# khanhptnk/psketch

Measured on AMD Instinct MI355X. Metric: env-steps/sec (whole node), 12x12 craft_medium, batch=65536, higher is better.
Workload: dtype fp32; 1 GPU; craft_medium_12x12_w3_B65536_random_rollout_full_features_K32; world=craft_medium_12x12, envs_per_gpu=65536, global_batch=65536, window=3, n_features=404, obs_dtype=fp32, state_dtype=u8 (exact small integers; the reference's float64 arrays hold the same values), obs_ring=16, pool=1024, parallelism=env-shard x1, ticks_per_launch=32, launches=81, teach_table=auto, obs_store=sc1, tile=32, rollout_threads=512

## Files before the change

psketch_amd/csrc/craft_episode.h:

```cpp
#pragma once
#include "craft_device.h"

namespace craft {


__device__ __forceinline__ int hashed_action(const SimView& v, uint64_t seed, int64_t slot, int64_t tick) {
  const uint64_t gid = (uint64_t)(v.env_base + slot);
  return (int)((uint32_t)(splitmix64(seed ^ (gid << 20) ^ (uint64_t)tick) >> 32) % 6u);
}

__device__ __forceinline__ bool state_in_range(const SimView& v, const Agent& s) {
  return !(s.x < 1 || s.x > v.W - 2 || s.y < 1 || s.y > v.H - 2 || s.scen >= v.pool_count);
}

__device__ __forceinline__ void protocol_step(Agent& s, const int& act, const uint32_t& flags, int& d, int& counted, bool& restart) {
  if (s.frozen) {
    d = 1;
  } else {
    counted = 1;
    s.timer -= 1;
    d = (act == CRAFT_STOP) || s.timer <= 0;
    restart = d && (flags & CRAFT_STEP_AUTORESET);
  }
}

__device__ __forceinline__ void language_step_begin(const Agent& s, const int& act, int& d, int& counted, bool& bad) {
  if (s.frozen) {
    d = 1;
  } else {
    bad = act < 0 || act >= CRAFT_N_ACTIONS;
    counted = !bad;
  }
}
__device__ __forceinline__ void language_step_end(Agent& s, const int& act, int& d) {
  s.timer -= 1;
  d = (act == CRAFT_STOP) || s.timer <= 0;
  if (d) {
    s.frozen = 1;
    s.timer = max(s.timer, 0);
  }
}

__device__ __forceinline__ void restart_agent(Agent& s, uint32_t init_word, int maxT) {
  s.x = init_word & 0xff; s.y = (init_word >> 8) & 0xff; s.dir = (init_word >> 16) & 3;
  s.timer = maxT;
}

__device__ __forceinline__ int32_t queue_next(int32_t cur, const uint32_t& count, const uint32_t& step, const uint32_t& wrap) {
  if (cur < 0) return -1;
  uint32_t nx = (uint32_t)cur + step;
  if (nx >= count) {
    if (!wrap) return -1;
    nx -= count;
  }
  return (int32_t)nx;
}

__device__ __forceinline__ bool episode_ends(const Agent& s, int act) {
  return !s.frozen && (act == CRAFT_STOP || s.timer <= 1);
}

__device__ __forceinline__ bool language_episode_ends(const Agent& s, int act) {
  return !s.frozen && act >= 0 && act < CRAFT_N_ACTIONS && (act == CRAFT_STOP || s.timer <= 1);
}

__device__ __forceinline__ void restart_from_entry(Agent& s, const uint2& e, int maxT) {
  s.scen = (int)(e.x & 0xffffffu);
  s.task = (int)(e.x >> 24);
  restart_agent(s, e.y, maxT);
}

__device__ __forceinline__ uint32_t pose_word(const Agent& s) {
  return (uint32_t)s.x | ((uint32_t)s.y << 8) | ((uint32_t)s.dir << 16);
}

template <int QB>
__device__ __forceinline__ void reload_grid_row(const uint4* pool_row, uint32_t* grid, const int& CS) {
  const int nchunk = CS >> 4;
#pragma unroll
  for (int b = 0; b < CRAFT_MAX_CELLS / 16; b += QB) {
    uint4 c[QB];
#pragma unroll
    for (int q = 0; q < QB; ++q)
      if (b + q < nchunk) c[q] = pool_row[b + q];
#pragma unroll
    for (int q = 0; q < QB; ++q)
      if (b + q < nchunk) {
        grid[4 * (b + q) + 0] = c[q].x; grid[4 * (b + q) + 1] = c[q].y;
        grid[4 * (b + q) + 2] = c[q].z; grid[4 * (b + q) + 3] = c[q].w;
      }
  }
}

__device__ __forceinline__ void freeze_agent(Agent& s) {
  s.frozen = 1;
  s.timer = max(s.timer, 0);
}

__device__ __forceinline__ int facing_cell(const Agent& s, int H) {
  return (s.x + dir_dx(s.dir)) * H + (s.y + dir_dy(s.dir));
}

__device__ __forceinline__ int satisfies_masked(const SimView& v, const uint8_t* g, const uint8_t* iv,
                                                const uint32_t (&m)[8], const Agent& s, uint32_t tt) {
  const int fc = facing_cell(s, v.H);
  uint32_t mw = 0;
#pragma unroll
  for (int w = 0; w < 8; ++w) mw |= (w == (fc >> 5)) ? m[w] : 0u;
  return satisfies_with(
      tt, [&](int arg) __attribute__((always_inline)) { return (int)iv[arg]; },
      [&]() __attribute__((always_inline)) { return ((mw >> (fc & 31)) & 1u) ? 0 : (int)g[fc]; });
}

__device__ __forceinline__ uint32_t agent_word(const Agent& s, bool live) {
  return live ? ((uint32_t)s.x | ((uint32_t)s.y << 8) | ((uint32_t)s.dir << 16) | (1u << 24)) : 0u;
}


__device__ __forceinline__ bool rewarded(const int& counted, const int& d, const int& succ) { return counted && d && succ == 1; }

template <class Args>
__device__ __forceinline__ void store_outputs(const Args& a, int64_t o, const int& d, const int& succ, const int& counted) {
  if (a.done) a.done[o] = (uint8_t)d;
  if (a.sat) a.sat[o] = (int8_t)succ;
  if (a.reward) a.reward[o] = rewarded(counted, d, succ) ? 1.0f : 0.0f;
}

__device__ __forceinline__ uint32_t pack_outputs(const int& d, const int& succ, const int& counted) {
  return (uint32_t)(uint8_t)d | ((uint32_t)(uint8_t)(int8_t)succ << 8) |
         ((uint32_t)rewarded(counted, d, succ) << 16) | (1u << 24);
}

__device__ __forceinline__ void tally_stats(const bool& live, const int& counted, const int& d, const int& succ,
                                            uint32_t& n_succ, uint32_t& n_end, uint32_t& n_step) {
  const uint64_t bs = __ballot(live && counted && d && succ == 1);
  const uint64_t be = __ballot(live && counted && d);
  const uint64_t bt = __ballot(live && counted);
  n_succ += (uint32_t)__popcll(bs);
  n_end += (uint32_t)__popcll(be);
  n_step += (uint32_t)__popcll(bt);
}
__device__ __forceinline__ void add_stats(const SimView& v, int64_t row, uint32_t n_succ, uint32_t n_end, uint32_t n_step) {
  unsigned long long* r = reinterpret_cast<unsigned long long*>(v.stats_part + 4 * row);
  atomicAdd(r + 0, (unsigned long long)n_succ);
  atomicAdd(r + 1, (unsigned long long)n_end);
  atomicAdd(r + 2, (unsigned long long)n_step);
}


template <class F>
__device__ __forceinline__ void for_each_masked_cell(const uint32_t (&m)[8], F f) {
#pragma unroll
  for (int w = 0; w < 8; ++w) {
    uint32_t mm = m[w];
    while (mm) {
      f(w * 32 + __ffs(mm) - 1);
      mm &= mm - 1;
    }
  }
}

__device__ __forceinline__ void apply_mask_to_row(const uint32_t (&m)[8], uint8_t* g) {
  for_each_masked_cell(m, [&](int c) __attribute__((always_inline)) { g[c] = 0; });
}


__device__ __forceinline__ void copy_row_words(uint32_t* dst, const uint32_t* src, const int& CS) {
  for (int q0 = 0; q0 < (CS >> 2); q0 += 12) {
    uint32_t w[12];
#pragma unroll
    for (int j = 0; j < 12; ++j) w[j] = q0 + j < (CS >> 2) ? src[q0 + j] : 0u;
#pragma unroll
    for (int j = 0; j < 12; ++j)
      if (q0 + j < (CS >> 2)) dst[q0 + j] = w[j];
  }
}

struct ClearList {
  uint32_t w = 0;
  __device__ __forceinline__ bool overflowed() const { return (w >> 31) != 0; }
  __device__ __forceinline__ uint32_t count() const { return (w >> 24) & 3; }
  __device__ __forceinline__ int cell(int i) const { return (int)((w >> (8 * i)) & 0xffu); }
  __device__ __forceinline__ bool has_room() const { return !overflowed() && count() < 3; }
  __device__ __forceinline__ void clear() { w = 0; }
  __device__ __forceinline__ void push(int c) {
    const uint32_t nc = count();
    w = overflowed() ? w
        : nc < 3 ? ((w & 0x00ffffffu) | ((uint32_t)c << (8 * nc)) | ((nc + 1) << 24)) : (1u << 31);
  }
  template <class K>
  __device__ __forceinline__ void restore(uint8_t* g, const uint32_t* pristine, const int& CS, K kind) const {
    if (overflowed()) {
      copy_row_words(reinterpret_cast<uint32_t*>(g), pristine, CS);
    } else {
      const int nc = (int)count();
#pragma unroll
      for (int i = 0; i < 3; ++i)
        if (i < nc) {
          const int c = cell(i);
          g[c] = kind(i, c);
        }
    }
  }
  __device__ __forceinline__ void restore(uint8_t* g, const uint32_t* pristine, const int& CS) const {
    const uint8_t* pr = reinterpret_cast<const uint8_t*>(pristine);
    restore(g, pristine, CS, [&](int, int c) __attribute__((always_inline)) { return pr[c]; });
  }
};

__device__ __forceinline__ void apply_mask_to_row(const uint32_t (&m)[8], uint8_t* g, ClearList& clr) {
  for_each_masked_cell(m, [&](int c) __attribute__((always_inline)) {
    g[c] = 0;
    clr.push(c);
  });
}

__device__ __forceinline__ void load_pool_row(const uint4* pool_row, uint32_t* pristine, uint32_t* grid, const int& CS) {
  const int nchunk = CS >> 4;
  for (int q0 = 0; q0 < nchunk; q0 += 4) {
    uint4 cq[4];
#pragma unroll
    for (int j = 0; j < 4; ++j)
      if (q0 + j < nchunk) cq[j] = pool_row[q0 + j];
#pragma unroll
    for (int j = 0; j < 4; ++j)
      if (q0 + j < nchunk) {
        const int q = 4 * (q0 + j);
        pristine[q + 0] = grid[q + 0] = cq[j].x;
        pristine[q + 1] = grid[q + 1] = cq[j].y;
        pristine[q + 2] = grid[q + 2] = cq[j].z;
        pristine[q + 3] = grid[q + 3] = cq[j].w;
      }
  }
}

__device__ __forceinline__ void cleared_mask(const uint32_t* pristine, const uint32_t* grid, const int& C, uint32_t (&m)[8]) {
#pragma unroll
  for (int i = 0; i < 8; ++i) m[i] = 0u;
#pragma unroll
  for (int q = 0; q < CRAFT_MAX_CELLS / 4; ++q)
    if (q < (C + 3) >> 2)
      m[q >> 3] |= byte_tops(nonzero_bytes(pristine[q]) & zero_bytes(grid[q])) << (4 * (q & 7));
}

__device__ __forceinline__ void publish_state(const SimView& v, const int64_t& slot, const uint64_t& st, const uint32_t* ivw,
                                              const uint32_t* m, bool sc1) {
  if (sc1) {
    typedef unsigned int u4v __attribute__((ext_vector_type(4)));
    const __amdgpu_buffer_rsrc_t inv_r = __builtin_amdgcn_make_buffer_rsrc(v.inv, 0, 0x7fffffff, 0x00020000);
    const __amdgpu_buffer_rsrc_t msk_r = __builtin_amdgcn_make_buffer_rsrc(v.mask, 0, 0x7fffffff, 0x00020000);
    const int off = (int)(slot * 32);
    __hip_atomic_store((gu64*)(v.state + slot), (unsigned long long)st, __ATOMIC_RELAXED,
                       __HIP_MEMORY_SCOPE_AGENT);
    __builtin_amdgcn_raw_buffer_store_b128(u4v{ivw[0], ivw[1], ivw[2], ivw[3]}, inv_r, off, 0, 16);
    __builtin_amdgcn_raw_buffer_store_b128(u4v{ivw[4], ivw[5], ivw[6], ivw[7]}, inv_r, off + 16, 0, 16);
    __builtin_amdgcn_raw_buffer_store_b128(u4v{m[0], m[1], m[2], m[3]}, msk_r, off, 0, 16);
    __builtin_amdgcn_raw_buffer_store_b128(u4v{m[4], m[5], m[6], m[7]}, msk_r, off + 16, 0, 16);
  } else {
    v.state[slot] = st;
    v.inv[2 * slot] = make_uint4(ivw[0], ivw[1], ivw[2], ivw[3]);
    v.inv[2 * slot + 1] = make_uint4(ivw[4], ivw[5], ivw[6], ivw[7]);
    v.mask[2 * slot] = make_uint4(m[0], m[1], m[2], m[3]);
    v.mask[2 * slot + 1] = make_uint4(m[4], m[5], m[6], m[7]);
  }
}

}
```

psketch_amd/csrc/craft_rollout_split.h:

```cpp
#pragma once
#include <type_traits>

#include "craft_episode.h"
#include "craft_obs.h"

namespace craft {

__host__ __device__ inline int split_stage_bytes(int tile, int CS) { return tile * (8 + 4 + 64) + tile * CS + tile * 40; }
__host__ __device__ inline int split_lds_bytes(int tile, int GS, int F, int CS, bool flat) {
  auto up16 = [](int x) { return (x + 15) & ~15; };
  return up16(3 * tile * GS) + 2 * up16(tile * F) + 2 * tile * kInvStride + 2 * tile * 4 +
         CRAFT_MAX_TASKS * 2 + CRAFT_MAX_RECIPES * 12 + 16 + 32 + 4 * tile * 4 +
         (flat ? split_stage_bytes(tile, CS) : 0);
}

template <int WIN, int TILE, int NT, int FMT, int WPE, bool GIVEN, bool FLAT = false, bool QUEUE = false>
__global__ __launch_bounds__(NT, WPE) void rollout_split_kernel(SimView v, RolloutArgs a) {
  extern __shared__ __attribute__((aligned(16))) uint8_t smem[];
  static_assert(!(QUEUE && FLAT), "the queue variant runs work units, one per tile");
  constexpr int DW = (WIN == 3 && TILE == 32 && NT == 512) ? 2 : 1;
  constexpr int E0 = 64 + 64 * DW;
  static_assert(NT >= E0 + 64 && TILE <= 64, "a producer, the scatter waves and at least one streaming wave");
  constexpr int P = 64 * DW / TILE;
  auto up16 = [](int x) { return (x + 15) & ~15; };
  const int GS = v.GS, F = v.F;
  const uint32_t rcv = v.rcw[min((int)(threadIdx.x & 63), CRAFT_MAX_RECIPES * 3 - 1)];
  uint8_t* s_grid = smem;
  uint8_t* s_pristine = smem + 2 * TILE * GS;
  const int obs_buf = up16(TILE * F);
  uint8_t* s_obs = smem + up16(3 * TILE * GS);
  uint8_t* s_inv = s_obs + 2 * obs_buf;
  uint32_t* s_agent = reinterpret_cast<uint32_t*>(s_inv + 2 * TILE * kInvStride);
  uint16_t* s_task = reinterpret_cast<uint16_t*>(s_agent + 2 * TILE);
  uint32_t* s_rc = reinterpret_cast<uint32_t*>(s_task + CRAFT_MAX_TASKS);
  uint32_t* s_ctrl = s_rc + CRAFT_MAX_RECIPES * 3;
  uint32_t* s_item = s_ctrl + 4;
  uint32_t* s_out = s_item + 8;
  uint8_t* s_stage = reinterpret_cast<uint8_t*>(s_out + 4 * TILE);

  const int tid = threadIdx.x;
  const int64_t n = v.n_envs;
  const bool want_obs = a.obs != nullptr;
  constexpr int esz = obs_elem_bytes(FMT);
  const int n_tiles = (int)((n + TILE - 1) / TILE);
  const int n_chunks = (a.n_ticks + a.chunk - 1) / a.chunk;
  const uint32_t n_units = (uint32_t)n_tiles * (uint32_t)n_chunks;

  Agent s{};
  uint64_t st = 0;
  uint32_t init_word = 0, task_word = 0;
  ClearList clr;
  ClearList clr_prev;
  uint32_t chg = 0;
  constexpr uint32_t kRestart = 0x80000000u;
  constexpr uint32_t kReload = 0x40000000u;
  int32_t cur = -1;
  uint2 qe = make_uint2(0u, 0u);
  int sync = 0;
  bool live = false;
  int64_t slot = 0;
  const uint32_t* pw = reinterpret_cast<const uint32_t*>(s_pristine + tid * GS);
  auto grid_of = [&](int p) __attribute__((always_inline)) { return s_grid + (p & 1) * TILE * GS + tid * GS; };
  auto inv_of = [&](int p) __attribute__((always_inline)) { return s_inv + (p & 1) * TILE * kInvStride + tid * kInvStride; };
  uint32_t n_succ = 0, n_end = 0, n_step = 0;

  auto tick_c = [&](int k, int p, bool lds_out) __attribute__((always_inline)) {
    const int64_t tick = a.tick0 + k;
    const int64_t r = tick % a.ring;
    int d = 0, succ = -1, counted = 0;
    uint8_t* g = grid_of(p);
    uint8_t* iv = inv_of(p);
    s = unpack_state(st);
    if (live) {
      if constexpr (QUEUE) {
        if (sync == 1 || chg == kReload)
          copy_row_words(reinterpret_cast<uint32_t*>(g), reinterpret_cast<const uint32_t*>(grid_of(p ^ 1)), v.CS);
        else if (chg) g[chg - 1] = 0;
      } else if (sync == 1) {
        copy_row_words(reinterpret_cast<uint32_t*>(g), reinterpret_cast<const uint32_t*>(grid_of(p ^ 1)), v.CS);
      } else if (sync == 2) {
        if (chg == kRestart) clr_prev.restore(g, pw, v.CS);
        else if (chg) g[chg - 1] = 0;
      }
      if (sync) {
        const uint32_t* src = reinterpret_cast<const uint32_t*>(inv_of(p ^ 1));
        uint32_t w[8];
#pragma unroll
        for (int i = 0; i < 8; ++i) w[i] = src[i];
#pragma unroll
        for (int i = 0; i < 8; ++i) reinterpret_cast<uint32_t*>(iv)[i] = w[i];
      }
      sync = sync ? 2 : 1;
      chg = 0;
      const int act = GIVEN ? a.actions[(int64_t)k * n + slot] : hashed_action(v, a.seed, slot, tick);
      bool restart = false;
      protocol_step(s, act, a.flags, d, counted, restart);
      if (d) succ = satisfies(v, g, iv, s, task_word);
      int32_t ended = -1, epose = -1;
      if constexpr (QUEUE) {
        if (restart) {
          ended = cur;
          epose = (int32_t)pose_word(s);
          cur = queue_next(cur, a.q_count, a.q_step, a.q_wrap);
          if (cur >= 0) {
            restart_from_entry(s, qe, v.maxT);
            task_word = s_task[s.task];
            init_word = qe.y;
#pragma unroll
            for (int w = 0; w < 8; ++w) reinterpret_cast<uint32_t*>(iv)[w] = 0u;
            load_pool_row(reinterpret_cast<const uint4*>(v.pool + (size_t)s.scen * v.CS),
                          reinterpret_cast<uint32_t*>(s_pristine + tid * GS), reinterpret_cast<uint32_t*>(g), v.CS);
            chg = kReload;
            const int32_t nxt = queue_next(cur, a.q_count, a.q_step, a.q_wrap);
            if (nxt >= 0) qe = a.q_entries[nxt];
          } else {
            freeze_agent(s);
          }
        }
      } else if (restart) {
        restart_agent(s, init_word, v.maxT);
#pragma unroll
        for (int w = 0; w < 8; ++w) reinterpret_cast<uint32_t*>(iv)[w] = 0u;
        clr.restore(g, pw, v.CS);
        clr_prev = clr;
        clr.clear();
        chg = kRestart;
      } else if (d && !s.frozen) {
        freeze_agent(s);
      }
      if (!d) {
        bool inv_changed = false, mask_changed = false;
        uint32_t m_unused[8] = {0, 0, 0, 0, 0, 0, 0, 0};
        const int fc = facing_cell(s, v.H);
        if (act < 0 || act >= CRAFT_N_ACTIONS) latch_error(v.err, CRAFT_EBADACTION, slot);
        else transition<true>(v, s_rc, g, iv, s, m_unused, act, inv_changed, mask_changed, rcv, slot);
        if (mask_changed) {
          chg = 1u + (uint32_t)fc;
          if constexpr (!QUEUE) clr.push(fc);
        }
      }
      st = pack_state(s);
      if (lds_out) s_out[(p & 3) * TILE + tid] = pack_outputs(d, succ, counted);
      else store_outputs(a, r * n + slot, d, succ, counted);
      if constexpr (QUEUE) {
        if (a.ep_end) a.ep_end[r * n + slot] = ended;
        if (a.end_pose) a.end_pose[r * n + slot] = epose;
        if (a.ep_now) a.ep_now[r * n + slot] = s.frozen ? -1 : cur;
      }
    } else if (lds_out && tid < TILE) {
      s_out[(p & 3) * TILE + tid] = 0u;
    }
    tally_stats(live, counted, d, succ, n_succ, n_end, n_step);
    s_agent[(p & 1) * TILE + tid] = agent_word(s, live);
  };

  uint64_t* sg_state = reinterpret_cast<uint64_t*>(s_stage);
  uint32_t* sg_init = reinterpret_cast<uint32_t*>(s_stage + TILE * 8);
  uint4* sg_inv = reinterpret_cast<uint4*>(s_stage + TILE * 12);
  uint4* sg_mask = reinterpret_cast<uint4*>(s_stage + TILE * 44);
  uint8_t* sg_pool = s_stage + TILE * 76;
  uint64_t* ob_state = reinterpret_cast<uint64_t*>(sg_pool + TILE * v.CS);
  uint32_t* ob_mask = reinterpret_cast<uint32_t*>(ob_state + TILE);

  auto load_tile = [&](int t, int p, auto STAGED) __attribute__((always_inline)) {
    constexpr bool staged = decltype(STAGED)::value;
    const int64_t env0 = (int64_t)t * TILE;
    const int nE = (int)min((int64_t)TILE, n - env0);
    slot = env0 + tid;
    live = tid < nE;
    uint32_t m[8] = {0, 0, 0, 0, 0, 0, 0, 0};
    uint32_t ivr[8] = {0, 0, 0, 0, 0, 0, 0, 0};
    if (live) {
      uint4 i0, i1, m0, m1;
      if constexpr (staged) {
        st = sg_state[tid];
        init_word = sg_init[tid];
        i0 = sg_inv[2 * tid]; i1 = sg_inv[2 * tid + 1];
        m0 = sg_mask[2 * tid]; m1 = sg_mask[2 * tid + 1];
      } else {
        st = v.state[slot];
        init_word = v.init[slot];
        if constexpr (QUEUE) cur = a.q_cursor[slot];
        i0 = v.inv[2 * slot]; i1 = v.inv[2 * slot + 1];
        m0 = v.mask[2 * slot]; m1 = v.mask[2 * slot + 1];
        if constexpr (QUEUE) {
          const int32_t nxt = queue_next(cur, a.q_count, a.q_step, a.q_wrap);
          if (nxt >= 0) qe = a.q_entries[nxt];
        }
      }
      ivr[0] = i0.x; ivr[1] = i0.y; ivr[2] = i0.z; ivr[3] = i0.w;
      ivr[4] = i1.x; ivr[5] = i1.y; ivr[6] = i1.z; ivr[7] = i1.w;
      m[0] = m0.x; m[1] = m0.y; m[2] = m0.z; m[3] = m0.w;
      m[4] = m1.x; m[5] = m1.y; m[6] = m1.z; m[7] = m1.w;
      s = unpack_state(st);
      if (!state_in_range(v, s)) {
        latch_error(v.err, CRAFT_EINVAL, slot);
        live = false;
      }
    }
    chg = 0;
    clr.clear();
    clr_prev.clear();
    sync = 0;
    if (live) {
      task_word = s_task[s.task];
      uint32_t* g0 = reinterpret_cast<uint32_t*>(grid_of(p));
      uint32_t* pwm = reinterpret_cast<uint32_t*>(s_pristine + tid * GS);
      const uint4* gsrc = reinterpret_cast<const uint4*>(v.pool + (size_t)s.scen * v.CS);
      const uint4* lsrc = reinterpret_cast<const uint4*>(sg_pool + tid * v.CS);
      const int nchunk = v.CS >> 4;
      if constexpr (staged) {
        for (int q0 = 0; q0 < nchunk; ++q0) {
          const uint4 c = lsrc[q0];
          const int q = 4 * q0;
          pwm[q + 0] = g0[q + 0] = c.x;
          pwm[q + 1] = g0[q + 1] = c.y;
          pwm[q + 2] = g0[q + 2] = c.z;
          pwm[q + 3] = g0[q + 3] = c.w;
        }
      } else {
        load_pool_row(gsrc, pwm, g0, v.CS);
      }
      uint32_t* iv0 = reinterpret_cast<uint32_t*>(inv_of(p));
#pragma unroll
      for (int i = 0; i < 8; ++i) iv0[i] = ivr[i];
      apply_mask_to_row(m, grid_of(p), clr);
    }
    __builtin_amdgcn_fence(__ATOMIC_RELEASE, "wavefront");
    __builtin_amdgcn_wave_barrier();
    __builtin_amdgcn_fence(__ATOMIC_ACQUIRE, "wavefront");
  };

  auto publish = [&](int p, bool sc1) __attribute__((always_inline)) {
    uint32_t m[8];
    cleared_mask(pw, reinterpret_cast<const uint32_t*>(grid_of(p)), v.C, m);
    publish_state(v, slot, st, reinterpret_cast<const uint32_t*>(inv_of(p)), m, sc1);
    if constexpr (QUEUE) {
      v.init[slot] = init_word;
      a.q_cursor[slot] = cur;
    }
  };

  auto scatter_d = [&](int p, int nE) __attribute__((always_inline)) {
    const int l = tid - 64, e = l % TILE;
    const uint32_t ag = s_agent[(p & 1) * TILE + e];
    if (e < nE && ag)
      scatter_env_part<WIN, P>(v, s_grid + (p & 1) * TILE * GS + e * GS,
                               s_inv + (p & 1) * TILE * kInvStride + e * kInvStride, ag,
                               s_obs + (p & 1) * obs_buf + e * F, l / TILE);
  };

  auto stream_e = [&](int p, int t, int k, bool outs) __attribute__((always_inline)) {
    const int64_t env0 = (int64_t)t * TILE;
    const int nE = (int)min((int64_t)TILE, n - env0);
    const int64_t r = (a.tick0 + k) % a.ring;
    if (outs && tid - E0 < nE) {
      const uint32_t w = s_out[(p & 3) * TILE + tid - E0];
      if (w >> 24) {
        const int64_t o = r * n + env0 + (tid - E0);
        if (a.done) a.done[o] = (uint8_t)(w & 0xffu);
        if (a.sat) a.sat[o] = (int8_t)((w >> 8) & 0xffu);
        if (a.reward) a.reward[o] = ((w >> 16) & 1u) ? 1.0f : 0.0f;
      }
    }
    void* out = static_cast<uint8_t*>(a.obs) + r * n * (int64_t)F * esz;
    stream_obs<FMT, NT - E0, true>(s_obs + (p & 1) * obs_buf, out, env0, F, nE, v.obs_policy, tid - E0);
  };

  for (int t = tid; t < v.n_tasks; t += NT) s_task[t] = v.task_tab[t];
  for (int t = tid; t < CRAFT_MAX_RECIPES * 3; t += NT) s_rc[t] = v.rcw[t];
  if (want_obs) {
    uint4* z = reinterpret_cast<uint4*>(s_obs);
    for (int i = tid; i < (2 * obs_buf >> 4); i += NT) z[i] = make_uint4(0, 0, 0, 0);
  }

  if constexpr (FLAT) {
#ifdef CRAFT_STAMPS
    unsigned long long t_beg = __builtin_amdgcn_s_memrealtime();
#define SPLIT_NOW() __builtin_amdgcn_s_memrealtime()
#else
#define SPLIT_NOW() 0ull
#endif
    unsigned long long acc_work = 0, acc_wait = 0, acc_sw = 0, acc_pub = 0, acc_vm = 0, acc_ld = 0, acc_dma = 0;
    int cur_t = -1, cur_k = 0;
    bool staged = false;
    auto stage_state = [&](int t2) __attribute__((always_inline)) {
      const int64_t e0 = (int64_t)t2 * TILE;
      const int l = tid;
      typedef __attribute__((address_space(1))) void* gp;
      typedef __attribute__((address_space(3))) void* lp;
      if (l < TILE / 2) __builtin_amdgcn_global_load_lds((gp)(v.state + e0 + 2 * l), (lp)sg_state, 16, 0, 0);
      if (l < TILE / 4) __builtin_amdgcn_global_load_lds((gp)(v.init + e0 + 4 * l), (lp)sg_init, 16, 0, 0);
#pragma unroll
      for (int h = 0; h < 2 * TILE; h += 64) {
        __builtin_amdgcn_global_load_lds((gp)(v.inv + 2 * e0 + h + l), (lp)(sg_inv + h), 16, 0, 0);
        __builtin_amdgcn_global_load_lds((gp)(v.mask + 2 * e0 + h + l), (lp)(sg_mask + h), 16, 0, 0);
      }
    };
    auto stage_pool = [&]() __attribute__((always_inline)) {
      typedef __attribute__((address_space(1))) void* gp;
      typedef __attribute__((address_space(3))) void* lp;
      const int per = v.CS >> 4;
      int e = tid / per, c = tid - (tid / per) * per;
      const int de = 64 / per, dc = 64 - (64 / per) * per;
      for (int f0 = 0; f0 < TILE * per; f0 += 64) {
        const int f = f0 + tid;
        if (f < TILE * per) {
          const int scen = (int)((sg_state[e] >> 32) & 0xffffffu) % max(1, v.pool_count);
          __builtin_amdgcn_global_load_lds((gp)(v.pool + (size_t)scen * v.CS + 16 * c), (lp)(sg_pool + 16 * f0),
                                           16, 0, 0);
        }
        e += de;
        c += dc;
        if (c >= per) { c -= per; ++e; }
      }
    };
    auto fetch_now = [&]() __attribute__((always_inline)) -> int {
      unsigned long long r = 0;
      if (tid == 0) r = atomicAdd(a.queue, 1ull);
      const uint32_t d = (uint32_t)__builtin_amdgcn_readfirstlane((int)(uint32_t)r) - (uint32_t)a.qbase;
      return d < (uint32_t)n_tiles ? (int)d : -1;
    };
    const int K = a.n_ticks;
    const int kF = max(0, K - 6), kA = max(0, K - 4), kB = max(0, K - 3);
    uint32_t pend = 0;
    int64_t pub_slot = -1;
    int t_next = -1;
    auto produce = [&](int j) __attribute__((always_inline)) {
      if (cur_t != -2 && (cur_t < 0 || cur_k == K)) {
        const unsigned long long s0 = SPLIT_NOW();
        const int t = cur_t == -1 ? fetch_now() : t_next;
        if (staged) asm volatile("s_waitcnt vmcnt(0)" ::: "memory");
        const unsigned long long s1 = SPLIT_NOW();
        const bool pub = cur_t >= 0 && tid < TILE && live;
        const int64_t pslot = slot;
        if (pub) {
          uint32_t m[8];
          cleared_mask(pw, reinterpret_cast<const uint32_t*>(grid_of(j - 1)), v.C, m);
          ob_state[tid] = st;
#pragma unroll
          for (int i = 0; i < 8; ++i) ob_mask[8 * tid + i] = m[i];
        }
        const unsigned long long s2 = SPLIT_NOW();
        if (t >= 0) {
          cur_t = t;
          cur_k = 0;
          if (tid < TILE) {
            if (staged) load_tile(t, j & 1, std::true_type{});
            else load_tile(t, j & 1, std::false_type{});
          }
        } else {
          cur_t = -2;
        }
        staged = false;
        t_next = -1;
        pub_slot = pub ? pslot : -1;
        const unsigned long long s3 = SPLIT_NOW();
        acc_sw += s3 - s0;
        acc_vm += s1 - s0;
        acc_pub += s2 - s1;
        acc_ld += s3 - s2;
      }
      const bool have = cur_t >= 0;
      if (have) {
        const unsigned long long d0 = SPLIT_NOW();
        if (cur_k == kF && tid == 0) pend = (uint32_t)atomicAdd(a.queue, 1ull);
        if (cur_k == kA) {
          const uint32_t d = (uint32_t)__builtin_amdgcn_readfirstlane((int)pend) - (uint32_t)a.qbase;
          t_next = d < (uint32_t)n_tiles ? (int)d : -1;
          if (t_next >= 0 && (int64_t)(t_next + 1) * TILE <= n) {
            asm volatile("s_waitcnt lgkmcnt(0)" ::: "memory");
            stage_state(t_next);
          }
        }
        if (cur_k == kB && t_next >= 0 && (int64_t)(t_next + 1) * TILE <= n) {
          asm volatile("s_waitcnt vmcnt(0)" ::: "memory");
          stage_pool();
          staged = true;
        }
        acc_dma += SPLIT_NOW() - d0;
      }
      if (have && tid < TILE) tick_c(cur_k, j, true);
      if (pub_slot >= 0) {
        publish_state(v, pub_slot, ob_state[tid], reinterpret_cast<const uint32_t*>(inv_of(j - 1)), ob_mask + 8 * tid, false);
        pub_slot = -1;
      }
      if (tid == 0) {
        s_item[2 * (j & 3)] = have ? (uint32_t)cur_t + 1u : 0u;
        s_item[2 * (j & 3) + 1] = (uint32_t)cur_k;
      }
      if (have) ++cur_k;
    };
    auto interval_end = [&](int i, unsigned long long w0) __attribute__((always_inline)) -> bool {
      const unsigned long long w1 = SPLIT_NOW();
      asm volatile("s_waitcnt lgkmcnt(0)" ::: "memory");
      __builtin_amdgcn_s_barrier();
      asm volatile("" ::: "memory");
      acc_work += w1 - w0;
      acc_wait += SPLIT_NOW() - w1;
      return s_item[2 * (i & 3)] == 0;
    };
    if (tid < 64) {
      produce(0);
      asm volatile("s_waitcnt lgkmcnt(0)" ::: "memory");
      __builtin_amdgcn_s_barrier();
      asm volatile("" ::: "memory");
      for (int i = 0;; ++i) {
        const unsigned long long w0 = SPLIT_NOW();
        produce(i + 1);
        if (interval_end(i, w0)) break;
      }
    } else if (tid < E0) {
      asm volatile("s_waitcnt lgkmcnt(0)" ::: "memory");
      __builtin_amdgcn_s_barrier();
      asm volatile("" ::: "memory");
      for (int i = 0;; ++i) {
        const unsigned long long w0 = SPLIT_NOW();
        const uint32_t t1 = s_item[2 * (i & 3)];
        if (t1) scatter_d(i & 1, (int)min((int64_t)TILE, n - (int64_t)(t1 - 1) * TILE));
        if (interval_end(i, w0)) break;
      }
    } else {
      asm volatile("s_waitcnt lgkmcnt(0)" ::: "memory");
      __builtin_amdgcn_s_barrier();
      asm volatile("" ::: "memory");
      for (int i = 0;; ++i) {
        const unsigned long long w0 = SPLIT_NOW();
        if (i >= 1) {
          const uint32_t t1 = s_item[2 * ((i - 1) & 3)];
          if (t1) stream_e(i - 1, (int)t1 - 1, (int)s_item[2 * ((i - 1) & 3) + 1], true);
        }
        if (interval_end(i, w0)) break;
      }
    }
#ifdef CRAFT_STAMPS
    if (v.stamps) {
      uint64_t* row = v.stamps + 16 * (int64_t)blockIdx.x;
      if (tid == 0) {
        row[0] = t_beg; row[1] = acc_work; row[2] = acc_wait; row[6] = SPLIT_NOW(); row[7] = acc_sw;
        row[8] = acc_vm; row[9] = acc_pub; row[10] = acc_ld; row[11] = acc_dma;
      } else if (tid == 64) {
        row[3] = acc_work; row[4] = acc_wait;
      } else if (tid == E0) {
        row[5] = acc_work;
      }
    }
#endif
    (void)acc_work;
    (void)acc_wait;
    (void)acc_sw;
    (void)acc_pub;
    (void)acc_vm;
    (void)acc_ld;
    (void)acc_dma;
#undef SPLIT_NOW
  } else {
    (void)s_out;
    (void)s_stage;
#ifdef CRAFT_STAMPS
    uint64_t* srow_t = v.stamps ? v.stamps + 16 * (int64_t)blockIdx.x : nullptr;
    if (tid == 0 && srow_t) srow_t[0] = __builtin_amdgcn_s_memrealtime();
    int n_done = 0;
#endif
    bool first = (uint32_t)blockIdx.x < n_units;
    for (;;) {
      if (tid == 0)
        s_ctrl[0] = first ? (uint32_t)blockIdx.x
                          : (uint32_t)(gridDim.x + (atomicAdd(a.queue + 1, 1ull) - a.qbase1));
      first = false;
      __syncthreads();
      const uint32_t u = s_ctrl[0];
#ifdef CRAFT_STAMPS
      if (tid == 0 && srow_t && n_done < 12) srow_t[1 + n_done] = __builtin_amdgcn_s_memrealtime();
#endif
      if (u >= n_units) break;
      const int t = (int)(u % (uint32_t)n_tiles), c = (int)(u / (uint32_t)n_tiles);
      const int k0 = c * a.chunk, k1 = min(a.n_ticks, k0 + a.chunk);
      const int nq = k1 - k0;
      const int64_t env0 = (int64_t)t * TILE;
      const int nE = (int)min((int64_t)TILE, n - env0);

      const bool state_only = a.ring >= a.n_ticks;
      const bool handoff = c + 1 < n_chunks;
      auto full_release = [&]() __attribute__((always_inline)) {
        asm volatile("s_waitcnt vmcnt(0)" ::: "memory");
        __syncthreads();
        if (tid == 0) {
          __builtin_amdgcn_fence(__ATOMIC_RELEASE, "agent");
          asm volatile("s_waitcnt vmcnt(0)" ::: "memory");
          __hip_atomic_store((gu32*)(a.tile_done + t), (uint32_t)(c + 1), __ATOMIC_RELAXED,
                             __HIP_MEMORY_SCOPE_AGENT);
        }
      };
      if (tid < 64) {
        if (c > 0) {
          bool ok = true;
          if (tid == 0) {
            const gu32* f = (const gu32*)(a.tile_done + t);
            for (uint32_t spins = 0; __hip_atomic_load(f, __ATOMIC_RELAXED, __HIP_MEMORY_SCOPE_AGENT) < (uint32_t)c;) {
              __builtin_amdgcn_s_sleep(2);
              if (++spins > (1u << 26)) { ok = false; break; }
            }
            if (!ok) latch_error(v.err, CRAFT_EINVARIANT, env0);
          }
          __builtin_amdgcn_fence(__ATOMIC_ACQUIRE, "agent");
        }
        if (tid < TILE) {
          load_tile(t, 0, std::false_type{});
          tick_c(k0, 0, false);
        }
        if (want_obs) {
          __syncthreads();
          for (int i = 0; i <= nq; ++i) {
            if (tid < TILE && i + 1 < nq) tick_c(k0 + i + 1, i + 1, false);
            __syncthreads();
          }
        } else if (tid < TILE) {
          for (int q = 1; q < nq; ++q) tick_c(k0 + q, q, false);
        }
        if (tid < TILE && live) publish(nq - 1, handoff && state_only);
        if (handoff && state_only) {
          asm volatile("s_waitcnt vmcnt(0)" ::: "memory");
          if (tid == 0)
            __hip_atomic_store((gu32*)(a.tile_done + t), (uint32_t)(c + 1), __ATOMIC_RELAXED,
                               __HIP_MEMORY_SCOPE_AGENT);
        } else if (handoff) {
          full_release();
        }
      } else {
        if (want_obs) {
          __syncthreads();
          if (tid < E0) {
#pragma unroll 1
            for (int i = 0; i <= nq; ++i) {
              if (i < nq) scatter_d(i, nE);
              __syncthreads();
            }
          } else {
            for (int i = 0; i <= nq; ++i) {
              if (i >= 1) stream_e(i - 1, t, k0 + i - 1, false);
#ifdef CRAFT_STAMPS
              if (tid == E0 && srow_t && n_done == 0 && i == 1) srow_t[13] = __builtin_amdgcn_s_memrealtime();
#endif
              __syncthreads();
            }
          }
        }
        if (handoff && !state_only) full_release();
      }
      __syncthreads();
#ifdef CRAFT_STAMPS
      ++n_done;
#endif
    }
#ifdef CRAFT_STAMPS
    if (tid == 0 && srow_t) {
      srow_t[14] = (uint64_t)n_done;
      srow_t[15] = __builtin_amdgcn_s_memrealtime();
    }
#endif
  }

  if (tid == 0) add_stats(v, (int64_t)blockIdx.x, n_succ, n_end, n_step);
}

}
```

Before: 3.615 billion env-steps/s.

## Move next-tile prefetch to scatter wave via registers and double-buffer pristine pool

Tile prefetch (queue claim, state/inventory/mask fetch, pool-row fetch) moves off the producer wave onto the first scatter wave. Data now goes through registers and lands in a pristine buffer that alternates with the staging pool, so the producer no longer copies staged rows into pristine. Handoff to the producer goes through s_ctrl words. Separately, the per-episode cleared mask is built from the clear list when it has not overflowed, avoiding a full-row pristine/grid compare at publish. The change adds register pressure on the scatter wave and new cross-wave synchronization through LDS control words.

```diff
diff --git a/psketch_amd/csrc/craft_episode.h b/psketch_amd/csrc/craft_episode.h
--- a/psketch_amd/csrc/craft_episode.h
+++ b/psketch_amd/csrc/craft_episode.h
@@ -215,6 +215,13 @@
   });
 }
 
+__device__ __forceinline__ void apply_mask_to_row_listed(const uint32_t (&m)[8], uint8_t* g, ClearList& clr) {
+  for_each_masked_cell(m, [&](int c) __attribute__((always_inline)) {
+    if (g[c]) clr.push(c);
+    g[c] = 0;
+  });
+}
+
 __device__ __forceinline__ void load_pool_row(const uint4* pool_row, uint32_t* pristine, uint32_t* grid, const int& CS) {
   const int nchunk = CS >> 4;
   for (int q0 = 0; q0 < nchunk; q0 += 4) {
@@ -241,6 +248,25 @@
   for (int q = 0; q < CRAFT_MAX_CELLS / 4; ++q)
     if (q < (C + 3) >> 2)
       m[q >> 3] |= byte_tops(nonzero_bytes(pristine[q]) & zero_bytes(grid[q])) << (4 * (q & 7));
+}
+
+__device__ __forceinline__ void list_mask(const ClearList& clr, uint32_t (&m)[8]) {
+#pragma unroll
+  for (int i = 0; i < 8; ++i) m[i] = 0u;
+  const int nc = (int)clr.count();
+#pragma unroll
+  for (int i = 0; i < 3; ++i) {
+    const int c = clr.cell(i);
+    const uint32_t bit = i < nc ? 1u << (c & 31) : 0u;
+#pragma unroll
+    for (int w = 0; w < 8; ++w) m[w] |= (c >> 5) == w ? bit : 0u;
+  }
+}
+
+__device__ __forceinline__ void episode_mask(const ClearList& clr, const uint32_t* pristine, const uint32_t* grid,
+                                             const int& C, uint32_t (&m)[8]) {
+  if (clr.overflowed()) cleared_mask(pristine, grid, C, m);
+  else list_mask(clr, m);
 }
 
 __device__ __forceinline__ void publish_state(const SimView& v, const int64_t& slot, const uint64_t& st, const uint32_t* ivw,
diff --git a/psketch_amd/csrc/craft_rollout_split.h b/psketch_amd/csrc/craft_rollout_split.h
--- a/psketch_amd/csrc/craft_rollout_split.h
+++ b/psketch_amd/csrc/craft_rollout_split.h
@@ -59,7 +59,8 @@
   int sync = 0;
   bool live = false;
   int64_t slot = 0;
-  const uint32_t* pw = reinterpret_cast<const uint32_t*>(s_pristine + tid * GS);
+  const uint32_t* pw = reinterpret_cast<const uint32_t*>(s_pristine + tid * (FLAT ? v.CS : GS));
+  int pbuf = 0;
   auto grid_of = [&](int p) __attribute__((always_inline)) { return s_grid + (p & 1) * TILE * GS + tid * GS; };
   auto inv_of = [&](int p) __attribute__((always_inline)) { return s_inv + (p & 1) * TILE * kInvStride + tid * kInvStride; };
   uint32_t n_succ = 0, n_end = 0, n_step = 0;
@@ -111,6 +112,7 @@
             load_pool_row(reinterpret_cast<const uint4*>(v.pool + (size_t)s.scen * v.CS),
                           reinterpret_cast<uint32_t*>(s_pristine + tid * GS), reinterpret_cast<uint32_t*>(g), v.CS);
             chg = kReload;
+            clr.clear();
             const int32_t nxt = queue_next(cur, a.q_count, a.q_step, a.q_wrap);
             if (nxt >= 0) qe = a.q_entries[nxt];
           } else {
@@ -136,7 +138,7 @@
         else transition<true>(v, s_rc, g, iv, s, m_unused, act, inv_changed, mask_changed, rcv, slot);
         if (mask_changed) {
           chg = 1u + (uint32_t)fc;
-          if constexpr (!QUEUE) clr.push(fc);
+          clr.push(fc);
         }
       }
       st = pack_state(s);
@@ -168,6 +170,11 @@
     const int nE = (int)min((int64_t)TILE, n - env0);
     slot = env0 + tid;
     live = tid < nE;
+    if constexpr (FLAT) {
+      pbuf ^= 1;
+      pw = reinterpret_cast<const uint32_t*>((pbuf ? sg_pool : s_pristine) + tid * v.CS);
+      if (tid == 0) s_ctrl[3] = (uint32_t)pbuf;
+    }
     uint32_t m[8] = {0, 0, 0, 0, 0, 0, 0, 0};
     uint32_t ivr[8] = {0, 0, 0, 0, 0, 0, 0, 0};
     if (live) {
@@ -205,18 +212,18 @@
     if (live) {
       task_word = s_task[s.task];
       uint32_t* g0 = reinterpret_cast<uint32_t*>(grid_of(p));
-      uint32_t* pwm = reinterpret_cast<uint32_t*>(s_pristine + tid * GS);
+      uint32_t* pwm = const_cast<uint32_t*>(pw);
       const uint4* gsrc = reinterpret_cast<const uint4*>(v.pool + (size_t)s.scen * v.CS);
-      const uint4* lsrc = reinterpret_cast<const uint4*>(sg_pool + tid * v.CS);
       const int nchunk = v.CS >> 4;
       if constexpr (staged) {
+        const uint4* lsrc = reinterpret_cast<const uint4*>(pw);
         for (int q0 = 0; q0 < nchunk; ++q0) {
           const uint4 c = lsrc[q0];
           const int q = 4 * q0;
-          pwm[q + 0] = g0[q + 0] = c.x;
-          pwm[q + 1] = g0[q + 1] = c.y;
-          pwm[q + 2] = g0[q + 2] = c.z;
-          pwm[q + 3] = g0[q + 3] = c.w;
+          g0[q + 0] = c.x;
+          g0[q + 1] = c.y;
+          g0[q + 2] = c.z;
+          g0[q + 3] = c.w;
         }
       } else {
         load_pool_row(gsrc, pwm, g0, v.CS);
@@ -224,7 +231,7 @@
       uint32_t* iv0 = reinterpret_cast<uint32_t*>(inv_of(p));
 #pragma unroll
       for (int i = 0; i < 8; ++i) iv0[i] = ivr[i];
-      apply_mask_to_row(m, grid_of(p), clr);
+      apply_mask_to_row_listed(m, grid_of(p), clr);
     }
     __builtin_amdgcn_fence(__ATOMIC_RELEASE, "wavefront");
     __builtin_amdgcn_wave_barrier();
@@ -233,7 +240,7 @@
 
   auto publish = [&](int p, bool sc1) __attribute__((always_inline)) {
     uint32_t m[8];
-    cleared_mask(pw, reinterpret_cast<const uint32_t*>(grid_of(p)), v.C, m);
+    episode_mask(clr, pw, reinterpret_cast<const uint32_t*>(grid_of(p)), v.C, m);
     publish_state(v, slot, st, reinterpret_cast<const uint32_t*>(inv_of(p)), m, sc1);
     if constexpr (QUEUE) {
       v.init[slot] = init_word;
@@ -283,37 +290,50 @@
 #endif
     unsigned long long acc_work = 0, acc_wait = 0, acc_sw = 0, acc_pub = 0, acc_vm = 0, acc_ld = 0, acc_dma = 0;
     int cur_t = -1, cur_k = 0;
-    bool staged = false;
-    auto stage_state = [&](int t2) __attribute__((always_inline)) {
+    static_assert(TILE == 32, "the continuous pipeline's prefetch: one inventory and one mask uint4 per lane");
+    constexpr int kPoolRegs = CRAFT_MAX_CELLS / 16 * TILE / 64;
+    uint64_t f_state = 0;
+    uint32_t f_init = 0;
+    uint4 f_inv = make_uint4(0, 0, 0, 0), f_mask = make_uint4(0, 0, 0, 0);
+    uint4 f_pool[kPoolRegs];
+#pragma unroll
+    for (int i = 0; i < kPoolRegs; ++i) f_pool[i] = make_uint4(0, 0, 0, 0);
+    auto fetch_state = [&](int t2, int l) __attribute__((always_inline)) {
       const int64_t e0 = (int64_t)t2 * TILE;
-      const int l = tid;
-      typedef __attribute__((address_space(1))) void* gp;
-      typedef __attribute__((address_space(3))) void* lp;
-      if (l < TILE / 2) __builtin_amdgcn_global_load_lds((gp)(v.state + e0 + 2 * l), (lp)sg_state, 16, 0, 0);
-      if (l < TILE / 4) __builtin_amdgcn_global_load_lds((gp)(v.init + e0 + 4 * l), (lp)sg_init, 16, 0, 0);
-#pragma unroll
-      for (int h = 0; h < 2 * TILE; h += 64) {
-        __builtin_amdgcn_global_load_lds((gp)(v.inv + 2 * e0 + h + l), (lp)(sg_inv + h), 16, 0, 0);
-        __builtin_amdgcn_global_load_lds((gp)(v.mask + 2 * e0 + h + l), (lp)(sg_mask + h), 16, 0, 0);
-      }
-    };
-    auto stage_pool = [&]() __attribute__((always_inline)) {
-      typedef __attribute__((address_space(1))) void* gp;
-      typedef __attribute__((address_space(3))) void* lp;
+      if (l < TILE) {
+        f_state = v.state[e0 + l];
+        f_init = v.init[e0 + l];
+      }
+      f_inv = v.inv[2 * e0 + l];
+      f_mask = v.mask[2 * e0 + l];
+    };
+    auto fetch_pool = [&](int l) __attribute__((always_inline)) {
+      if (l < TILE) {
+        sg_state[l] = f_state;
+        sg_init[l] = f_init;
+      }
+      sg_inv[l] = f_inv;
+      sg_mask[l] = f_mask;
       const int per = v.CS >> 4;
-      int e = tid / per, c = tid - (tid / per) * per;
+      int e = l / per, c = l - (l / per) * per;
       const int de = 64 / per, dc = 64 - (64 / per) * per;
-      for (int f0 = 0; f0 < TILE * per; f0 += 64) {
-        const int f = f0 + tid;
-        if (f < TILE * per) {
+#pragma unroll
+      for (int i = 0; i < kPoolRegs; ++i) {
+        if (64 * i + l < TILE * per) {
           const int scen = (int)((sg_state[e] >> 32) & 0xffffffu) % max(1, v.pool_count);
-          __builtin_amdgcn_global_load_lds((gp)(v.pool + (size_t)scen * v.CS + 16 * c), (lp)(sg_pool + 16 * f0),
-                                           16, 0, 0);
+          f_pool[i] = reinterpret_cast<const uint4*>(v.pool + (size_t)scen * v.CS)[c];
         }
         e += de;
         c += dc;
         if (c >= per) { c -= per; ++e; }
       }
+    };
+    auto land_pool = [&](int l, uint32_t pb) __attribute__((always_inline)) {
+      uint4* pnext = reinterpret_cast<uint4*>(pb ? s_pristine : sg_pool);
+      const int per = v.CS >> 4;
+#pragma unroll
+      for (int i = 0; i < kPoolRegs; ++i)
+        if (64 * i + l < TILE * per) pnext[64 * i + l] = f_pool[i];
     };
     auto fetch_now = [&]() __attribute__((always_inline)) -> int {
       unsigned long long r = 0;
@@ -322,21 +342,40 @@
       return d < (uint32_t)n_tiles ? (int)d : -1;
     };
     const int K = a.n_ticks;
-    const int kF = max(0, K - 6), kA = max(0, K - 4), kB = max(0, K - 3);
+    const bool ahead = K >= 2;
+    const int cF = max(0, K - 7), cA = max(0, K - 5), cB = max(0, K - 4), cW = K - 2;
     uint32_t pend = 0;
+    int t_next = -1;
+    bool fetching = false;
+    auto prefetch = [&](int k) __attribute__((always_inline)) {
+      const int l = tid - 64;
+      if (k == cF && l == 0) pend = (uint32_t)atomicAdd(a.queue, 1ull);
+      if (k == cA) {
+        const uint32_t d = (uint32_t)__builtin_amdgcn_readfirstlane((int)pend) - (uint32_t)a.qbase;
+        t_next = d < (uint32_t)n_tiles ? (int)d : -1;
+        fetching = t_next >= 0 && (int64_t)(t_next + 1) * TILE <= n;
+        if (l == 0) {
+          s_ctrl[1] = (uint32_t)(t_next + 1);
+          s_ctrl[2] = fetching ? 1u : 0u;
+        }
+        if (fetching) fetch_state(t_next, l);
+      }
+      if (k == cB && fetching) fetch_pool(l);
+      if (k == cW && fetching) land_pool(l, (uint32_t)__builtin_amdgcn_readfirstlane((int)s_ctrl[3]));
+    };
     int64_t pub_slot = -1;
-    int t_next = -1;
     auto produce = [&](int j) __attribute__((always_inline)) {
       if (cur_t != -2 && (cur_t < 0 || cur_k == K)) {
         const unsigned long long s0 = SPLIT_NOW();
-        const int t = cur_t == -1 ? fetch_now() : t_next;
-        if (staged) asm volatile("s_waitcnt vmcnt(0)" ::: "memory");
+        const bool claimed = cur_t >= 0 && ahead;
+        const int t = claimed ? __builtin_amdgcn_readfirstlane((int)s_ctrl[1]) - 1 : fetch_now();
+        const bool staged = claimed && __builtin_amdgcn_readfirstlane((int)s_ctrl[2]) != 0;
         const unsigned long long s1 = SPLIT_NOW();
         const bool pub = cur_t >= 0 && tid < TILE && live;
         const int64_t pslot = slot;
         if (pub) {
           uint32_t m[8];
-          cleared_mask(pw, reinterpret_cast<const uint32_t*>(grid_of(j - 1)), v.C, m);
+          episode_mask(clr, pw, reinterpret_cast<const uint32_t*>(grid_of(j - 1)), v.C, m);
           ob_state[tid] = st;
 #pragma unroll
           for (int i = 0; i < 8; ++i) ob_mask[8 * tid + i] = m[i];
@@ -352,8 +391,6 @@
         } else {
           cur_t = -2;
         }
-        staged = false;
-        t_next = -1;
         pub_slot = pub ? pslot : -1;
         const unsigned long long s3 = SPLIT_NOW();
         acc_sw += s3 - s0;
@@ -362,24 +399,6 @@
         acc_ld += s3 - s2;
       }
       const bool have = cur_t >= 0;
-      if (have) {
-        const unsigned long long d0 = SPLIT_NOW();
-        if (cur_k == kF && tid == 0) pend = (uint32_t)atomicAdd(a.queue, 1ull);
-        if (cur_k == kA) {
-          const uint32_t d = (uint32_t)__builtin_amdgcn_readfirstlane((int)pend) - (uint32_t)a.qbase;
-          t_next = d < (uint32_t)n_tiles ? (int)d : -1;
-          if (t_next >= 0 && (int64_t)(t_next + 1) * TILE <= n) {
-            asm volatile("s_waitcnt lgkmcnt(0)" ::: "memory");
-            stage_state(t_next);
-          }
-        }
-        if (cur_k == kB && t_next >= 0 && (int64_t)(t_next + 1) * TILE <= n) {
-          asm volatile("s_waitcnt vmcnt(0)" ::: "memory");
-          stage_pool();
-          staged = true;
-        }
-        acc_dma += SPLIT_NOW() - d0;
-      }
       if (have && tid < TILE) tick_c(cur_k, j, true);
       if (pub_slot >= 0) {
         publish_state(v, pub_slot, ob_state[tid], reinterpret_cast<const uint32_t*>(inv_of(j - 1)), ob_mask + 8 * tid, false);
@@ -418,6 +437,11 @@
         const unsigned long long w0 = SPLIT_NOW();
         const uint32_t t1 = s_item[2 * (i & 3)];
         if (t1) scatter_d(i & 1, (int)min((int64_t)TILE, n - (int64_t)(t1 - 1) * TILE));
+        if (tid < 128 && t1 && ahead) {
+          const unsigned long long d0 = SPLIT_NOW();
+          prefetch((int)s_item[2 * (i & 3) + 1]);
+          acc_dma += SPLIT_NOW() - d0;
+        }
         if (interval_end(i, w0)) break;
       }
     } else {
@@ -438,9 +462,9 @@
       uint64_t* row = v.stamps + 16 * (int64_t)blockIdx.x;
       if (tid == 0) {
         row[0] = t_beg; row[1] = acc_work; row[2] = acc_wait; row[6] = SPLIT_NOW(); row[7] = acc_sw;
-        row[8] = acc_vm; row[9] = acc_pub; row[10] = acc_ld; row[11] = acc_dma;
+        row[8] = acc_vm; row[9] = acc_pub; row[10] = acc_ld;
       } else if (tid == 64) {
-        row[3] = acc_work; row[4] = acc_wait;
+        row[3] = acc_work; row[4] = acc_wait; row[11] = acc_dma;
       } else if (tid == E0) {
         row[5] = acc_work;
       }
```

Result: no change. 3.605 billion env-steps/s (-0.3%).
